# jynik/OOKiedokie

Hardware: AMD Instinct MI355X
Metric: IQ Msamples/s demodulated (SC16Q11->bits) (higher is better)
Workload: dtype f32

## Files before the change

### ookiedokie_amd/build.py

```python
from __future__ import annotations

import os
import shutil
import subprocess
import sys

HERE = os.path.dirname(os.path.abspath(__file__))
CSRC = os.path.join(HERE, "csrc")
LIB = os.path.join(HERE, "lib", "libookiedokie_amd.so")
SOURCES = ["loaders.cpp", "front_plan.cpp", "rx.cpp", "synth.cpp", "stream_fir.cpp", "backend.cpp", "edges_fsm.hip", "fsm_scan.hip",
           "formatter.cpp", "kernels.hip", "fir_mfma.hip", "fir_tuned.hip", "scan_ctx.cpp", "survey.cpp", "survey.hip",
           "survey_tuned.hip", "spectrum.cpp", "spectrum.hip", "pulses.cpp", "pulses.hip"]
ARCH = "gfx950"


def _hipcc() -> str:
    for cand in (shutil.which("hipcc"), "/opt/rocm/bin/hipcc"):
        if cand and os.path.exists(cand):
            return cand
    raise RuntimeError("hipcc not found")


def sources():
    return [os.path.join(CSRC, s) for s in SOURCES if os.path.exists(os.path.join(CSRC, s))]


def needs_build() -> bool:
    if not os.path.exists(LIB):
        return True
    t = os.path.getmtime(LIB)
    deps = sources() + [os.path.join(CSRC, f) for f in os.listdir(CSRC) if f.endswith(".hpp")]
    deps.append(os.path.join(HERE, "..", "include", "ookiedokie_amd.h"))
    return any(os.path.getmtime(d) > t for d in deps)


def build(force: bool = False, verbose: bool = False) -> str:
    if not force and not needs_build():
        return LIB
    os.makedirs(os.path.dirname(LIB), exist_ok=True)
    objs = []
    for src in sources():
        obj = os.path.join(HERE, "lib", os.path.basename(src) + ".o")
        cmd = [_hipcc(), "-x", "hip", "--offload-arch=" + ARCH, "-O3", "-std=c++17", "-fPIC",
               "-ffp-contract=off", "-fno-fast-math", "-Wall", "-Wno-unused-result", "-Wno-uninitialized",
               "-mllvm", "-amdgpu-atomic-optimizer-strategy=None",
               "-c", src, "-o", obj]
        if verbose:
            print(" ".join(cmd))
        r = subprocess.run(cmd, capture_output=True, text=True)
        if r.returncode != 0:
            raise RuntimeError("hipcc failed on %s:\n%s%s" % (src, r.stdout, r.stderr))
        if verbose and r.stderr:
            print(r.stderr)
        objs.append(obj)
    cmd = [_hipcc(), "--offload-arch=" + ARCH, "-shared", "-fPIC", "-o", LIB] + objs
    r = subprocess.run(cmd, capture_output=True, text=True)
    if r.returncode != 0:
        raise RuntimeError("link failed:\n%s%s" % (r.stdout, r.stderr))
    return LIB


if __name__ == "__main__":
    print(build(force="--force" in sys.argv, verbose=True))
```

### ookiedokie_amd/csrc/edges_fsm.hip

```cpp
#include "kernels.hpp"

namespace ookd {

__device__ __forceinline__ uint32_t lane_id() { return threadIdx.x & 63u; }

__device__ __forceinline__ uint32_t rfl(uint32_t v) {
    return (uint32_t)__builtin_amdgcn_readfirstlane((int)v);
}
__device__ __forceinline__ uint64_t rfl64(uint64_t v) {
    return ((uint64_t)rfl((uint32_t)(v >> 32)) << 32) | rfl((uint32_t)v);
}
__device__ __forceinline__ uint32_t rl(uint32_t v, uint32_t lane) {
    return (uint32_t)__builtin_amdgcn_readlane((int)v, (int)lane);
}
__device__ __forceinline__ uint64_t rl64(uint64_t v, uint32_t lane) {
    return ((uint64_t)rl((uint32_t)(v >> 32), lane) << 32) | rl((uint32_t)v, lane);
}


__device__ __forceinline__ uint64_t change_word(const uint64_t *words, uint64_t w, uint64_t n_out, uint32_t has_prev = 0) {
    const uint64_t cur = words[w];
    const uint64_t prev_top = (w == 0 && !has_prev) ? 0ull : (*(words + w - 1) >> 63);
    const uint64_t e = cur ^ ((cur << 1) | prev_top);
    const uint64_t base = w * 64;
// ... 67 lines not shown
#pragma unroll
    for (int d = 1; d < 64; d <<= 1) {
        const uint32_t t = __shfl_up(inc, d);
        if ((int)lane_id() >= d) inc += t;
    }
    if (lane_id() == 63) wave_sum[tid >> 6] = inc;
    __syncthreads();
    uint32_t before = 0;
    for (uint32_t w = 0; w < (tid >> 6); ++w) before += wave_sum[w];
    uint32_t run = before + inc - mine;
    if (quad && ((uintptr_t)(p.blk_offset + base) & 15u) == 0) {
        *reinterpret_cast<uint4 *>(p.blk_offset + base) = make_uint4(run, run + v[0], run + v[0] + v[1], run + v[0] + v[1] + v[2]);
        run += mine;
    } else {
#pragma unroll
        for (int i = 0; i < 4; ++i) {
            if (base + i < n) p.blk_offset[base + i] = run;
            run += v[i];
        }
    }
    if (tid == 255) p.group_total[blockIdx.x] = run;
}

__global__ __launch_bounds__(1024) void edge_scan_groups_kernel(const EdgeParams p) {
    __builtin_amdgcn_s_setprio(3);
    __shared__ uint32_t wtot[16];
    const uint32_t n = p.num_captures * p.blocks_per_cap;
    const uint32_t ng = (n + kScanGroup - 1) / kScanGroup;
    const uint32_t tid = threadIdx.x;
    const uint32_t chunk = (ng + 1023u) / 1024u;
    const uint32_t lo = min(tid * chunk, ng);
    const uint32_t hi = min(lo + chunk, ng);
    uint32_t sum = 0;
    for (uint32_t i = lo; i < hi; ++i) sum += p.group_total[i];
    uint32_t total = 0;
    uint32_t run = wg_inclusive_sum(sum, wtot, &total) - sum;
    for (uint32_t i = lo; i < hi; ++i) {
        const uint32_t t = p.group_total[i];
        p.group_total[i] = run;
        run += t;
    }
    if (tid == 1023) {
        p.blk_offset[n] = total;
        if ((uint64_t)total > p.edge_capacity) *p.overflow = 1;
        if (p.total_acc) atomicAdd(p.total_acc, total);
    }
}

constexpr uint32_t kWriteSpan = 4;

__global__ __launch_bounds__(256) void edge_write_kernel(const EdgeParams p) {
    __builtin_amdgcn_s_setprio(3);
    const uint32_t wave = (blockIdx.x * blockDim.x + threadIdx.x) >> 6;
    const uint32_t lane = lane_id();
    const uint32_t total_blocks = p.num_captures * p.blocks_per_cap;
    const uint32_t nwaves = (total_blocks + kWriteSpan - 1) / kWriteSpan;
    if (wave >= nwaves) return;
    uint32_t off = 0, cnt = 0;
    if (lane < kWriteSpan && wave + lane * nwaves < total_blocks) {
        const uint32_t b = wave + lane * nwaves;
        off = p.blk_offset[b] + p.group_total[b / kScanGroup];
        p.blk_offset[b] = off;
        cnt = p.blk_count[b];
    }
    uint64_t todo = __ballot(cnt != 0);
// ... 803 lines not shown
    }
    if (tid < p.hdr_words) {
        uint32_t v = p.d_hdr[tid];
        if (tid == p.edges_word && p.total_edges) v = *p.total_edges;
        p.h_hdr[tid] = v;
    }
    __syncthreads();
    if (tid < p.hdr_words) p.d_hdr[tid] = 0;
}

hipError_t launch_publish(const PublishParams &p, hipStream_t stream) {
    hipLaunchKernelGGL(publish_kernel, dim3(1), dim3(256), 0, stream, p);
    return hipGetLastError();
}


hipError_t launch_edges(const EdgeParams &p, hipStream_t stream) {
    const uint32_t total_blocks = p.num_captures * p.blocks_per_cap;
    if (total_blocks == 0) return hipSuccess;
    const uint32_t wgs = (total_blocks + 3) / 4;
    const uint32_t groups = (total_blocks + kScanGroup - 1) / kScanGroup;
    if (!p.tile_info) hipLaunchKernelGGL(edge_count_kernel, dim3(wgs), dim3(256), 0, stream, p);
    hipLaunchKernelGGL(edge_scan_local_kernel, dim3(groups), dim3(256), 0, stream, p);
    hipLaunchKernelGGL(edge_scan_groups_kernel, dim3(1), dim3(1024), 0, stream, p);
    if (p.tile_info) {
        const dim3 grid((uint32_t)(((uint64_t)total_blocks * p.tiles_per_block + 255) / 256));
        if (p.tiles_per_block == 4) hipLaunchKernelGGL(edge_write_tiles_kernel<4>, grid, dim3(256), 0, stream, p);
        else if (p.tiles_per_block == 8) hipLaunchKernelGGL(edge_write_tiles_kernel<8>, grid, dim3(256), 0, stream, p);
        else if (p.tiles_per_block == 16) hipLaunchKernelGGL(edge_write_tiles_kernel<16>, grid, dim3(256), 0, stream, p);
        else return hipErrorInvalidValue;
    } else {
        const uint32_t write_waves = (total_blocks + kWriteSpan - 1) / kWriteSpan;
        hipLaunchKernelGGL(edge_write_kernel, dim3((write_waves + 3) / 4), dim3(256), 0, stream, p);
    }
    return hipGetLastError();
}

hipError_t launch_fsm_prepare(const FsmParams &p, const FsmStateDev *first_state, hipStream_t stream) {
    const uint32_t nseg = p.num_captures * p.segs_per_cap;
    if (nseg == 0) return hipSuccess;
    FsmStateDev first{};
    if (first_state) first = *first_state;
    hipLaunchKernelGGL(fsm_cuts_kernel, dim3(p.num_captures * (p.segs_per_cap + 1)), dim3(64), 0, stream, p);
    hipLaunchKernelGGL(fsm_prepare_kernel, dim3((nseg + 63) / 64), dim3(64), 0, stream, p, first,
                       first_state ? 1 : 0);
    return hipGetLastError();
}
// ... 23 lines not shown
```

### ookiedokie_amd/csrc/fir_mfma.hip

```cpp
#include "kernels.hpp"
#include "common.hpp"

#include <hip/hip_ext.h>

#include <algorithm>
#include <cmath>
#include <cstring>
#include <type_traits>

#pragma clang fp contract(off)

namespace ookd {

typedef _Float16 h8 __attribute__((ext_vector_type(8)));
typedef _Float16 h4 __attribute__((ext_vector_type(4)));
typedef float f16x __attribute__((ext_vector_type(16)));
typedef float v2fm __attribute__((ext_vector_type(2)));
typedef short v2s __attribute__((ext_vector_type(2)));
typedef uint32_t v4u __attribute__((ext_vector_type(4)));

__host__ __device__ constexpr uint32_t mslot(uint32_t j) { return j + 8u * (j >> 5); }

template <int KS, int FMT = (int)kFmtSc16>
struct MfmaGeom {
// ... 505 lines not shown

        if (!more) break;
        if (!pre) mfma_boundary_loads<KS, FMT>(c, tile_n, tid, win, q);
        tile = tile_n;
    }
}

constexpr uint32_t kF2Out = 256;
constexpr uint32_t kF2Tp = 96;
constexpr uint32_t kF2W = 4 * kF2Out + kF2Tp;
template <int FMT>
struct F2Geom {
    static constexpr uint32_t vsamples = FMT == (int)kFmtSc16 ? 4u : 8u;
    static constexpr uint32_t nvec = kF2W / vsamples;
    static constexpr int rounds = (int)((nvec + 63) / 64);
};
constexpr int kF2KS = 5;
constexpr int kF2Waves = 4;
__host__ __device__ constexpr uint32_t f2slot(uint32_t j) { return j + 8u * (j >> 6); }
constexpr uint32_t kF2Plane = f2slot(kF2W) + 8u;
constexpr uint32_t kF2WaveBytes = kF2Plane * 2u * 2u;
constexpr uint32_t kF2ImgBytes = kF2KS * 2u * 1024u;
constexpr uint32_t kF2LdsBytes = kF2ImgBytes + kMfmaCtlBytes + kF2Waves * kF2WaveBytes;

typedef float f4x __attribute__((ext_vector_type(4)));

struct F2Taps {
    gptrf taps1, taps2;
    uint32_t n1, n2;
};

template <int FMT>
__device__ __forceinline__ float2 fir2_mfma_exact_output(const RawSrcT<FMT> &rs, const F2Taps &ft, int64_t m) {
    const float s = 1.0f / 2048.0f;
    float re2 = 0.0f, im2 = 0.0f;
    for (uint32_t k2 = 0; k2 < ft.n2; ++k2) {
        const int64_t j1 = 2 * m + 1 - (int64_t)k2;
        float re1 = 0.0f, im1 = 0.0f;
        for (uint32_t k1 = 0; k1 < ft.n1; ++k1) {
            const uint32_t w = fetch_raw_m(rs, 2 * j1 + 1 - (int64_t)k1);
            const float xr = (float)(int16_t)(w & 0xffffu) * s;
            const float xi = (float)(int16_t)(w >> 16) * s;
            const float t = ft.taps1[k1];
            const float pr = t * xr;
            const float pi = t * xi;
            re1 = re1 + pr;
// ... 532 lines not shown
```

### ookiedokie_amd/csrc/fsm_scan.hip

```cpp
#include "kernels.hpp"
#include "common.hpp"

#include <hip/hip_ext.h>

#include <algorithm>
#include <cstring>
#include <memory>
#include <vector>

namespace ookd {

namespace {

enum { kCondAlways = 1, kCondPulseStart, kCondPulseEnd, kCondTimeout, kCondMsgComplete };
enum { kActNone = 1, kActAppend0, kActAppend1, kActOutput };
enum { kResError = -1, kResNone = 0, kResOutput = 1 };

constexpr uint32_t kNone = 0xffffffffu;
constexpr uint32_t kSat = 0xfffffffeu;
constexpr uint32_t kMaxFires = 48;
constexpr uint32_t kMaxLeafApps = 30;
constexpr int kScanThreads = 1024;
constexpr uint32_t kStuckDepth = 8;
constexpr uint32_t kStuckDomain = 512;
// ... 292 lines not shown
    f.k = r.w[1];
    f.nbits = r.w[2];
    a.reset_seen = (r.w[0] >> 10) & 1u;
    a.sensitive = (r.w[0] >> 11) & 1u;
    a.overflow = (r.w[0] >> 12) & 1u;
    a.last_fired = (r.w[0] >> 14) & 1u;
    a.msgc_seen = (r.w[0] >> 13) & 1u;
    a.napp = r.w[3] & 0xffu;
    a.nout = (r.w[3] >> 8) & 0xffu;
    a.nerr = (r.w[3] >> 16) & 0xffu;
    a.apps_at_reset = r.w[3] >> 24;
    a.appvals = r.w[4];
    a.out_ab0 = r.w[5] & 0xffu;
    a.out_ab1 = (r.w[5] >> 8) & 0xffu;
    a.out_rb0 = (r.w[5] >> 16) & 0xffu;
    a.out_rb1 = r.w[5] >> 24;
    a.out_pos0 = r.w[6] | ((uint64_t)r.w[7] << 32);
    a.out_pos1 = r.w[8] | ((uint64_t)r.w[9] << 32);
    a.err_pos = r.w[10] | ((uint64_t)r.w[11] << 32);
    a.fires = 0;
    return (r.w[0] >> 9) & 1u;
}

__host__ __device__ __noinline__ SimRes run_leaf_raw(const LTab &T, uint32_t code, uint64_t pos0, uint64_t n, uint32_t lvl_edge,
                                            uint64_t resume, uint64_t prefix = 0) {
    const uint32_t NB1 = T.NB1;
    const uint32_t nstates = T.S * NB1;
    const uint32_t L = lvl_edge & 1u;
    const bool has_edge = (lvl_edge & 2u) != 0;
    PSim f;
    Acc a;
    acc_init(a);
    bool alive;
    if (code >= nstates) {
        f.cur = 0;
        f.nbits = 0;
        f.k = 0;
        f.prev = code - nstates;
        const uint64_t end_const = pos0 + n;
        const uint64_t last = end_const + (has_edge ? 1 : 0);
        if (resume >= last) alive = false;
        else if (resume >= end_const) alive = sim_span(T, f, a, resume, L, 0, has_edge);
        else alive = sim_span(T, f, a, resume, L, end_const - resume, has_edge);
    } else {
        f.cur = code / NB1;
        f.nbits = code - f.cur * NB1;
        f.k = 0;
        f.prev = L;
        bool lost = false;
        if (prefix) {
            lost = !sim_span(T, f, a, pos0 - prefix, L, prefix, false) || a.overflow;
            acc_init(a);
        }
        alive = sim_span(T, f, a, pos0, L, n, has_edge);
        if (lost) a.overflow = true;
    }
    return sim_pack(f, a, alive);
}

__device__ __forceinline__ bool run_leaf(const LTab &T, uint32_t code, const Span &sp, uint64_t resume, PSim &f,
                                         Acc &a) {
    const SimRes r = run_leaf_raw(T, code, sp.pos0, sp.n, sp.L | (sp.has_edge ? 2u : 0u), resume, sp.prefix);
    return sim_unpack(r, f, a);
}

__host__ __device__ __forceinline__ uint32_t encode_post(const LTab &T, const PSim &f, const Acc &a, bool alive) {
    if (a.overflow) return code_poison(T);
    if (!alive) return code_skip(T, f.prev);
    if (f.k != 0 && !(T.st[f.cur].w & 0x10000u)) return code_poison(T);
    return f.cur * T.NB1 + (f.nbits >= T.NB1 ? T.NB1 - 1 : f.nbits);
}

}

struct ScanParams {
    FsmParams f;
    uint16_t *block_tab;
    uint32_t *cap_block_off;
    LeafEvDev *events;
    uint8_t *app_vals;
    uint64_t app_capacity;
    uint64_t *errs;
    uint64_t err_capacity;
    FsmStateDev first;
    int have_first;
// ... 741 lines not shown
        STAMP(3);
#pragma unroll
        for (int j = 0; j < kIlp; ++j)
            if (valid[j]) row[code[j]] = (uint16_t)st[j];
    }
    STAMP(4);
    bool any = false;
    for (uint32_t w = 0; w < kCapWords; ++w) any = any || cap[w] != 0;
    if (any && T.NS) {
        const uint32_t nst = T.NS * T.depth;
        for (uint32_t item = threadIdx.x; item < nch * nst; item += blockDim.x) {
            const uint32_t c = item / nst, code = D0 + (item - c * nst);
            const uint32_t la = c * kChunk, lb = min((c + 1) * kChunk, count);
            const uint32_t ob = la + kStuckDepth - ((code - D0) / T.NS + 1);
            if (!(cap[ob >> 5] & (1u << (ob & 31u)))) continue;
            uint32_t v = code;
            for (uint32_t l = la; l < lb; ++l) v = leaf_step(T, sc, first, b.tab, rep, skip, SNB, l, v);
            b.ctab[c * D + code] = (uint16_t)v;
        }
    }
    __syncthreads();
}

__global__ __launch_bounds__(kScanThreads) void scan_layout_kernel(ScanParams sp) {
    __builtin_amdgcn_s_setprio(3);
    __shared__ uint32_t wtot[kScanThreads / 64];
    const uint32_t tid = threadIdx.x;
    const uint32_t nc = sp.f.num_captures;
    const uint32_t chunk = (nc + kScanThreads - 1) / kScanThreads;
    const uint32_t lo = min(tid * chunk, nc), hi = min(lo + chunk, nc);
    uint32_t sum = 0, sum2 = 0, sum3 = 0, sum4 = 0;
    for (uint32_t c = lo; c < hi; ++c) {
        uint64_t e0;
        const uint64_t ne = cap_edges(sp.f, c, e0);
        const uint64_t regular = ne > 1 ? ne - 1 : 0;
        const uint32_t nblk = (uint32_t)((regular + sp.leaf_block - 1) / sp.leaf_block);
        sum += nblk;
        sum2 += (uint32_t)((ne + 1 + kFinBlock - 1) / kFinBlock);
        sum3 += (nblk + 15u) / 16u;
        sum4 += (nblk + 63u) / 64u;
    }
    uint32_t tot = 0, tot2 = 0, tot3 = 0, tot4 = 0;
    uint32_t run = wg_inclusive_sum(sum, wtot, &tot) - sum;
    uint32_t run2 = wg_inclusive_sum(sum2, wtot, &tot2) - sum2;
    uint32_t run3 = wg_inclusive_sum(sum3, wtot, &tot3) - sum3;
    uint32_t run4 = wg_inclusive_sum(sum4, wtot, &tot4) - sum4;
    for (uint32_t c = lo; c < hi; ++c) {
        sp.cap_block_off[c] = run;
        sp.fin_off[c] = run2;
        sp.cap_group_off[c] = run3;
        sp.cap_super_off[c] = run4;
        uint64_t e0;
        const uint64_t ne = cap_edges(sp.f, c, e0);
        const uint64_t regular = ne > 1 ? ne - 1 : 0;
        const uint32_t nblk = (uint32_t)((regular + sp.leaf_block - 1) / sp.leaf_block);
        run += nblk;
        run2 += (uint32_t)((ne + 1 + kFinBlock - 1) / kFinBlock);
        run3 += (nblk + 15u) / 16u;
        run4 += (nblk + 63u) / 64u;
    }
    if (tid == kScanThreads - 1) {
        sp.cap_block_off[nc] = tot;
        sp.fin_off[nc] = tot2;
        sp.cap_group_off[nc] = tot3;
        sp.cap_super_off[nc] = tot4;
        if (tot > sp.total_blocks_cap || tot2 > sp.fin_blocks_cap) atomicOr(sp.fallback, (uint32_t)kFbBlocks);
        if (sp.edge_overflow && *sp.edge_overflow) atomicOr(sp.fallback, (uint32_t)kFbBlocks);
    }
}

__global__ __launch_bounds__(kSimThreads) void scan_leaf_kernel(ScanParams sp) {
    __builtin_amdgcn_s_setprio(3);
    __shared__ LTab T;
    __shared__ uint64_t s_resume[256];
    __shared__ uint16_t s_rep[256], s_uniq[258];
    __shared__ __attribute__((aligned(4))) uint16_t s_skip[256][2];
    __shared__ uint32_t s_cap[kCapWords];
    __shared__ uint32_t s_lt[kLtLdsWords];
    copy_ltab(T, sp.ltab);
    __syncthreads();
    if (threadIdx.x == 0) T.lvl0 = sp.has_prev ? fsm_level_at(sp.f, 0, -1) : 0u;
    __syncthreads();
    if (*sp.fallback) return;
    const uint32_t D = T.D, LB = sp.leaf_block;
// ... 1029 lines not shown
                    }
                }
            }
            if (bad && !stop && sp.f.debug) sp.f.debug[63] = gb | ((uint64_t)lb << 32);
            reinterpret_cast<uint16_t *>(rec + kSyncRecEnd)[k] = (uint16_t)s;
            if (bad) atomicOr(sp.sync_fail, 1u);
            mine = (arrive | (stop ? 0u : 4u)) << (3u * k);
        }
        mine |= (uint32_t)__shfl_xor((int)mine, 1);
        mine |= (uint32_t)__shfl_xor((int)mine, 2);
        mine |= (uint32_t)__shfl_xor((int)mine, 4);
        if (region && k == 0) sp.sync_dig[gb] = (info & 0x7fu) | 0x80u | (info & 0x700u) | (mine << kSyncDigMap);
    }
}

__device__ __forceinline__ uint32_t sync_map_identity() { return 0x03020100u; }
__device__ __forceinline__ uint32_t sync_map_apply(uint32_t m, uint32_t x) { return (m >> (8u * x)) & 0xffu; }
__device__ __forceinline__ uint32_t sync_map_then(uint32_t a, uint32_t b) {
    uint32_t r = 0;
#pragma unroll
    for (uint32_t x = 0; x < kSyncK; ++x) r |= sync_map_apply(b, sync_map_apply(a, x) & 3u) << (8u * x);
    return r;
}
constexpr uint32_t kPickPer = 32;

__device__ __forceinline__ uint32_t sync_dig_map(uint32_t dig) {
    const uint32_t mb = dig >> kSyncDigMap;
    return (mb & 3u) | (((mb >> 3) & 3u) << 8) | (((mb >> 6) & 3u) << 16) | (((mb >> 9) & 3u) << 24);
}

__global__ __launch_bounds__(kScanThreads) void scan_syncpick_kernel(ScanParams sp) {
    __builtin_amdgcn_s_setprio(3);
    __shared__ uint32_t maps[2][kScanThreads / 64];
    __shared__ uint32_t lastc[kScanThreads];
    uint32_t *const dig = reinterpret_cast<uint32_t *>(scan_smem);
    const uint32_t tid = threadIdx.x;
    if (*sp.fallback) return;
    if (*sp.sync_fail & 1u) {
        if (sp.sync_only && tid == 0) atomicOr(sp.fallback, (uint32_t)kFbSync);
        return;
    }
    for (uint32_t cap = blockIdx.x; cap < sp.f.num_captures; cap += gridDim.x) {
        const uint32_t gb0 = sp.cap_block_off[cap], nblk = sp.cap_block_off[cap + 1] - gb0;
        const uint32_t per = (nblk + kScanThreads - 1) / kScanThreads;
        if (per > kPickPer) {
            if (tid == 0) {
                atomicOr(sp.sync_fail, 1u);
                if (sp.sync_only) atomicOr(sp.fallback, (uint32_t)kFbSync);
            }
            return;
        }
        for (uint32_t i = tid; i < nblk; i += kScanThreads) dig[i] = sp.sync_dig[gb0 + i];
        __syncthreads();
        const uint32_t b0 = min(tid * per, nblk), b1 = min(b0 + per, nblk);
        uint32_t m = sync_map_identity();
        for (uint32_t b = b0; b < b1; ++b) {
            const uint32_t d = dig[b];
            if (d & 0x80u) m = sync_map_then(m, sync_dig_map(d));
        }
        const uint32_t lane = tid & 63u, wv = tid >> 6;
        uint32_t incl = m;
#pragma unroll
        for (uint32_t d = 1; d < 64; d <<= 1) {
            const uint32_t other = (uint32_t)__shfl_up((int)incl, (int)d);
            if (lane >= d) incl = sync_map_then(other, incl);
        }
        if (lane == 63) maps[0][wv] = incl;
        __syncthreads();
        if (wv == 0) {
            uint32_t t = lane < (uint32_t)(kScanThreads / 64) ? maps[0][lane] : sync_map_identity();
#pragma unroll
            for (uint32_t d = 1; d < (uint32_t)(kScanThreads / 64); d <<= 1) {
                const uint32_t other = (uint32_t)__shfl_up((int)t, (int)d);
                if (lane >= d) t = sync_map_then(other, t);
            }
            if (lane < (uint32_t)(kScanThreads / 64)) maps[1][lane] = t;
        }
        __syncthreads();
        uint32_t excl = (uint32_t)__shfl_up((int)incl, 1);
        if (lane == 0) excl = sync_map_identity();
        if (wv) excl = sync_map_then(maps[1][wv - 1], excl);
        uint32_t c = sync_map_apply(excl, 0u) & 3u;
        uint32_t last = 0xffffffffu;
        for (uint32_t b = b0; b < b1; ++b) {
            const uint32_t d = dig[b];
            if (d & 0x80u) {
                last = c;
                const uint32_t me = (d >> (kSyncDigMap + 3u * c)) & 7u;
                if (me & 4u) {
                    const uint32_t e = sp.sync_rec[(size_t)(gb0 + b) * kSyncRecWords + kSyncRecEnd + (c >> 1)];
                    sp.cap_end[cap] = (uint16_t)((e >> (16u * (c & 1u))) & 0xffffu);
                }
                dig[b] = (d & 0xffu) | (c << 12);
                c = me & 3u;
            } else {
                dig[b] = 64u;
            }
        }
        lastc[tid] = last;
        __syncthreads();
        uint32_t before = 0;
        if (b0 < b1) {
            for (uint32_t t = tid; t-- > 0;) {
                if (lastc[t] != 0xffffffffu) {
                    before = lastc[t];
                    break;
                }
            }
        }
        for (uint32_t b = b0; b < b1; ++b) {
            const uint32_t d = dig[b];
            dig[b] = (d & 0x7fu) | (before << 8) | (d & 0x3000u);
            if (d & 0x80u) before = (d >> 12) & 3u;
        }
        __syncthreads();
        for (uint32_t i = tid; i < nblk; i += kScanThreads) sp.sync_sel[gb0 + i] = dig[i];
        __syncthreads();
    }
}


__device__ __forceinline__ void emit_simulate(const ScanParams &sp, const LTab &T, uint32_t cap, const uint64_t *edges,
                                              size_t ev0, uint64_t i, uint32_t in) {
    const uint64_t e_before = edges[i - 1], e_at = edges[i];
    PSim f;
    Acc a;
    bool alive = true;
    if (in == code_poison(T)) {
        scan_refuse(sp, cap, (uint32_t)kFbPoison);
        acc_init(a);
        f.cur = f.nbits = f.k = f.prev = 0;
    } else {
        Span span;
        span.pos0 = e_before + 1;
        span.n = e_at - e_before - 1;
        span.L = (uint32_t)(i & 1ull) ^ T.lvl0;
        span.has_edge = true;
        span.prefix = 0;
        if (in >= T.S * T.NB1 + 3) {
            uint32_t d, src;
            stuck_decode(T, in, d, src);
            span.prefix = e_before - edges[i - d - 1];
            in = src;
        }
        alive = run_leaf(T, in, span, next_buffer_start(T, e_before), f, a);
        if (a.overflow) scan_refuse(sp, cap, (uint32_t)kFbOverflow);
    }
    put_event(sp, ev0 + i, a, f, alive, false);
}

constexpr uint32_t kEmitQueue = 1024;
struct EmitQ {
    uint32_t cap, in;
    uint64_t i;
};

__global__ __launch_bounds__(kSimThreads) void scan_emit_kernel(ScanParams sp) {
    __builtin_amdgcn_s_setprio(3);
    __shared__ LTab T;
    __shared__ EmitQ s_q[kEmitQueue];
    __shared__ uint32_t s_qn;
    copy_ltab(T, sp.ltab);
    __syncthreads();
    if (threadIdx.x == 0) {
        T.lvl0 = sp.has_prev ? fsm_level_at(sp.f, 0, -1) : 0u;
        s_qn = 0;
    }
    __syncthreads();
    if (*sp.fallback) return;
    const bool sync_form = sp.sync_try && !(*sp.sync_fail & 1u);
    const uint32_t LB = sp.leaf_block;
    const uint32_t total = sp.cap_block_off[sp.f.num_captures];
    if (sync_form) {
        const uint32_t r2 = sp.lt_merged[3] + 2u * (sp.lt_merged[0] + sp.lt_merged[1]);
        const uint32_t n2 = (sp.lt_merged[0] + sp.lt_merged[1]) * 2u * T.S;
        for (uint32_t i = threadIdx.x; i < n2; i += blockDim.x) g_mr[i] = sp.lt_merged[r2 + i];
        __syncthreads();
    }
    const uint32_t nquad = (total + 3u) / 4u;
    for (uint32_t wq = blockIdx.x; wq < nquad + sp.f.num_captures; wq += gridDim.x) {
// ... 81 lines not shown
                tail.prefix = 0;
                tail.pos0 = pos0;
                tail.n = sp.f.n_out > pos0 ? sp.f.n_out - pos0 : 0;
                tail.L = (uint32_t)(ne & 1ull) ^ T.lvl0;
                tail.has_edge = false;
                if (in > code_poison(T)) {
                    uint32_t d, src;
                    stuck_decode(T, in, d, src);
                    if (ne >= (uint64_t)d + 1) {
                        tail.prefix = edges[ne - 1] - edges[ne - d - 1];
                        in = src;
                    } else {
                        in = code_poison(T);
                    }
                }
                PSim f;
                Acc a;
                bool alive = true;
                if (in == code_poison(T)) {
                    scan_refuse(sp, cap, (uint32_t)kFbPoison);
                    acc_init(a);
                    f.cur = f.nbits = f.k = f.prev = 0;
                } else {
                    alive = run_leaf(T, in, tail, next_buffer_start(T, edges[ne - 1]), f, a);
                    if (a.overflow) scan_refuse(sp, cap, (uint32_t)kFbOverflow);
                }
                put_event(sp, ev0 + ne, a, f, alive, true);
            }
            __syncthreads();
        }
    }
    __syncthreads();
    const uint32_t nq = min(s_qn, kEmitQueue);
    for (uint32_t j = threadIdx.x; j < nq; j += blockDim.x) {
        const EmitQ e = s_q[j];
        uint64_t e0;
        (void)cap_edges(sp.f, e.cap, e0);
        emit_simulate(sp, T, e.cap, sp.f.edges + e0, (size_t)e0 + e.cap, e.i, e.in);
    }
}


__device__ __forceinline__ void locate_fin(const ScanParams &sp, uint32_t gfb, uint32_t &cap, uint32_t &fb) {
    uint32_t lo = 0, hi = sp.f.num_captures;
    while (hi - lo > 1) {
        const uint32_t mid = (lo + hi) >> 1;
        if (sp.fin_off[mid] <= gfb) lo = mid;
// ... 807 lines not shown
    sp.cap_super_off = a.cap_super_off;
    sp.super_tab = a.super_tab;
    sp.super_in = a.super_in;
    sp.sync_rec = a.sync_rec;
    sp.sync_dig = a.sync_rec ? a.sync_rec + (size_t)(a.total_blocks_cap + 8) * kSyncRecWords : nullptr;
    sp.sync_sel = a.sync_rec ? sp.sync_dig + a.total_blocks_cap + 8 : nullptr;
    sp.sync_fail = a.sync_fail;
    sp.sync_try = 0;
    sp.pre_plane = a.pre_plane;
    sp.lt_sync_words = a.lt_sync_words;
    sp.cap_end = a.cap_end;
    sp.cap_first = a.cap_first;
    const size_t lds = block_lds_bytes(a.leaf_block, a.D, a.S, a.SNB);
    const size_t lds_group = groups_lds_bytes(sp.Dp);
    const size_t lds_walk = (size_t)128 * sp.Dp * 2;
    if (lds_walk > 150u * 1024u) return hipErrorInvalidValue;
    hipError_t e;
    e = ensure_dynamic_lds(reinterpret_cast<const void *>(&scan_leaf_kernel), lds);
    if (e != hipSuccess) return e;
    e = ensure_dynamic_lds(reinterpret_cast<const void *>(&scan_walk_kernel), lds_walk);
    if (e != hipSuccess) return e;
    e = ensure_dynamic_lds(reinterpret_cast<const void *>(&scan_groups_kernel), lds_group);
    if (e != hipSuccess) return e;
    const size_t lds_pick = (size_t)kPickPer * kScanThreads * 4;
    e = ensure_dynamic_lds(reinterpret_cast<const void *>(&scan_syncpick_kernel), lds_pick);
    if (e != hipSuccess) return e;
    const char *const leaf_env = dev_getenv("OOKD_SCAN_LEAF");
    const size_t lds_wave = wave_lds_bytes(a.D, a.S);
    const bool wave_form = a.lt_off && a.lt_words && a.lt_words <= kLtLdsWords && a.leaf_block == 64 && lds_wave <= 60u * 1024u &&
                           !(leaf_env && leaf_env[0] == 'b');
    if (wave_form) {
        e = ensure_dynamic_lds(reinterpret_cast<const void *>(&scan_leaf_wave_kernel), lds_wave);
        if (e != hipSuccess) return e;
    }
    const uint32_t caps = a.f.num_captures;
    const uint32_t cap_grid = caps < 256 ? caps : 256;
    static thread_local int sim_dev = -1;
    static thread_local uint32_t leaf_grid = 0, emit_grid = 0, wave_grid = 0;
    static thread_local size_t wave_lds_seen = ~(size_t)0;
    if (wave_form) {
        int dev = 0;
        (void)hipGetDevice(&dev);
        if (dev != sim_dev || lds_wave != wave_lds_seen) {
            int per_cu = 0;
            hipDeviceProp_t prop;
            if (hipOccupancyMaxActiveBlocksPerMultiprocessor(&per_cu, scan_leaf_wave_kernel, 64, lds_wave) == hipSuccess &&
                hipGetDeviceProperties(&prop, dev) == hipSuccess && prop.multiProcessorCount > 0 && per_cu > 0) {
// ... 17 lines not shown
                hipGetDeviceProperties(&prop, dev) == hipSuccess && prop.multiProcessorCount > 0) {
                const int cus = prop.multiProcessorCount;
                leaf_grid = per_cu_leaf > 0 ? (uint32_t)(per_cu_leaf * cus) : a.grid_blocks;
                emit_grid = per_cu_emit > 0 ? (uint32_t)(per_cu_emit * cus) : a.grid_blocks;
            } else {
                (void)hipGetLastError();
                leaf_grid = emit_grid = a.grid_blocks;
            }
            sim_dev = dev;
            sim_lds = lds;
        }
    }
    static const char *const grid_env = dev_getenv("OOKD_SCAN_GRID");
    const uint32_t leaf_blocks = grid_env ? (uint32_t)atoi(grid_env) : leaf_grid;
    const uint32_t emit_blocks = grid_env ? (uint32_t)atoi(grid_env) : emit_grid;
    sp.skipc = wave_form ? a.skipc : nullptr;
    sp.skipc_valid = sp.skipc ? 1u : 0u;
    sp.pre_codes = a.pre_codes;
    sp.blk_in = a.blk_in;
    sp.rowz = a.rowz;
    sp.sync_try = (a.sync_try && wave_form && a.lt_merged && a.lt_sync_words && a.lt_sync_words <= kMergedLdsWords && a.rowz && a.skipc &&
                   a.pre_codes && a.pre_plane && a.sync_rec && a.sync_fail) ? 1u : 0u;
    sp.sync_only = sp.sync_try && a.sync_try == 2 ? 1u : 0u;
    hipLaunchKernelGGL(scan_layout_kernel, dim3(1), dim3(kScanThreads), 0, stream, sp);
    if (sp.sync_try) {
        hipLaunchKernelGGL(scan_sync_kernel, dim3(512), dim3(256), 0, stream, sp);
        hipLaunchKernelGGL(scan_syncwalk_kernel, dim3(512), dim3(256), 0, stream, sp);
        hipLaunchKernelGGL(scan_syncpick_kernel, dim3(cap_grid), dim3(kScanThreads), lds_pick, stream, sp);
    }
    if (!(sp.sync_try && sp.sync_only)) {
        if (wave_form) {
            hipLaunchKernelGGL(scan_leaf_wave_kernel, dim3(grid_env ? (uint32_t)atoi(grid_env) : wave_grid), dim3(64), lds_wave, stream, sp);
        } else {
            hipLaunchKernelGGL(scan_leaf_kernel, dim3(leaf_blocks), dim3(kSimThreads), lds, stream, sp);
        }
        hipLaunchKernelGGL(scan_groups_kernel, dim3(512), dim3(kGroupsThreads), lds_group, stream, sp);
        hipLaunchKernelGGL(scan_walk_kernel, dim3(cap_grid), dim3(kScanThreads), lds_walk, stream, sp);
        sp.entry_phase = 0;
        const bool with_phase2 = a.lt_off && a.lt_merged && a.rowz;
        hipLaunchKernelGGL(scan_entry_kernel, dim3(kEntryP0Blocks + (with_phase2 ? 512u : 0u)), dim3(256), 0, stream, sp);
        sp.entry_phase = 1;
        hipLaunchKernelGGL(scan_entry_kernel, dim3(512), dim3(256), 0, stream, sp);
    }
    hipLaunchKernelGGL(scan_emit_kernel, dim3(emit_blocks), dim3(kSimThreads), 0, stream, sp);
    hipLaunchKernelGGL(fin_write_kernel, dim3(256), dim3(kFinBlock), 0, stream, sp);
    hipExtLaunchKernelGGL(fin_msg_kernel, dim3(64), dim3(256), 0, stream, nullptr, t_end, 0, sp, a.publish);
    return hipGetLastError();
}

}
```

### ookiedokie_amd/csrc/kernels.hpp

```cpp
#pragma once

#include <hip/hip_runtime.h>

#include <vector>

#include <cstdint>

namespace ookd {

constexpr int kMaxStages = 8;
constexpr int kTapChunk = 32;
constexpr int kTunedChunk = 16;
constexpr int kFirThreads = 256;
constexpr int kFirR = 16;
constexpr int kFirTile = kFirThreads * kFirR;
constexpr int kFirWaves = kFirThreads / 64;
constexpr int kFirWgWaves = 1;
constexpr int kFir1RShort = 8, kFir1RLong = 16;
constexpr uint32_t kFir1ShortTaps = 256;
constexpr int kWaveTile = 64 * kFirR;
constexpr int kQuietCounters = 1024;
constexpr int kGenTile = 1024;
constexpr int kGenTileMin = 64;
constexpr size_t kGenLdsBytes = 160 * 1024;
// ... 114 lines not shown
bool front_uses_tuned_fir1(const FrontParams &p);
uint32_t tuned_fir1_tile_bits(const FrontParams &p);
hipError_t launch_front_tuned_fir1(const FrontParams &p, uint32_t num_captures, hipStream_t stream, hipEvent_t t0,
                                   hipEvent_t t1, uint64_t tile_begin, uint64_t tile_count);
hipError_t launch_front_tuned_generic(const FrontParams &p, uint32_t num_captures, hipStream_t stream);
constexpr uint32_t kMaxCarriers = 16;
struct TunedCarrierDev {
    uint32_t tap_off;
    float p_star, p_lo, p_hi;
    float quiet_a, quiet_b;
    uint32_t pad[2];
};
hipError_t launch_front_tuned_multi(const FrontParams &p, const TunedCarrierDev *carriers, uint32_t num_carriers,
                                    hipStream_t stream, hipEvent_t t0, hipEvent_t t1, uint64_t tile_begin,
                                    uint64_t tile_count);
hipError_t launch_front_generic(const FrontParams &p, uint32_t num_captures,
                                hipStream_t stream);
struct GenTile {
    uint32_t tile = 0;
    uint32_t lds_b_off = 0;
    uint64_t lds_bytes = 0;
};
GenTile generic_tile(const FirStageDev *stage, uint32_t num_stages);


constexpr int kScanGroup = 1024;

struct EdgeParams {
    const uint64_t *bits;
    uint64_t words_per_cap;
    uint64_t n_out;
    uint32_t num_captures;
    uint32_t blocks_per_cap;
    uint32_t *blk_count;
    uint32_t *blk_offset;
    uint32_t *group_total;
    uint64_t *edges;
    uint64_t edge_capacity;
    uint32_t *overflow;
    const uint32_t *tile_info;
    uint32_t tiles_per_block;
    uint32_t *total_acc;
    uint32_t has_prev;
    uint32_t stamp_bits;
};

// ... 170 lines not shown
    uint64_t pre_plane;
    uint32_t lt_sync_words;
    uint32_t *sync_fail;
    uint32_t sync_try;
};

constexpr uint32_t kScanFbSync = 16;
struct ScanTables {
    bool spans_built;
    uint32_t S, max_bits, NB1, SNB, D, leaf_block;
    std::vector<uint32_t> off, n0, pk;
    std::vector<uint16_t> reach;
    std::vector<uint16_t> reach_by_level;
    uint32_t reach_base, reach_lv[2];
    std::vector<uint16_t> stuck_src;
    std::vector<uint8_t> stuck_rows;
    std::vector<uint32_t> merged;
    uint32_t merged_rows_words;
    std::vector<uint4> ltab;
};
ScanTables build_scan_tables(const FsmTablesDev &tables, uint32_t spb, uint32_t decim, bool with_spans);
bool scan_tables_selfcheck(const ScanTables &t);
uint32_t fsm_scan_fin_block();
hipError_t launch_fsm_scan(const FsmScanArgs &a, hipStream_t stream, hipEvent_t t_end = nullptr);

#ifdef __HIPCC__
__device__ __forceinline__ uint32_t wg_inclusive_sum(uint32_t v, uint32_t *wtot, uint32_t *total) {
    const uint32_t lane = threadIdx.x & 63u, wave = threadIdx.x >> 6, nwaves = (blockDim.x + 63u) >> 6;
#pragma unroll
    for (int d = 1; d < 64; d <<= 1) {
        const uint32_t t = __shfl_up(v, d);
        if ((int)lane >= d) v += t;
    }
    __syncthreads();
    if (lane == 63u || threadIdx.x == blockDim.x - 1) wtot[wave] = v;
    __syncthreads();
    uint32_t before = 0, all = 0;
    for (uint32_t w = 0; w < nwaves; ++w) {
        const uint32_t t = wtot[w];
        if (w < wave) before += t;
        all += t;
    }
    if (total) *total = all;
    return v + before;
}
#endif
// ... 95 lines not shown
```

Measured before the change: 1.555 million.

## Shrink single-block scan kernels to a shared slot size so they co-reside with front-end

Introduces a 'slot' budget (256 threads, 128 VGPRs, LDS left after three front-end workgroups) and resizes the edge group scan, scan layout and sync-pick kernels from 1024/kScanThreads threads to this slot. Sync-pick is restructured into multiple passes with carried map state so its LDS footprint fits the slot, and scan_emit gets a VGPR cap. The intent is to let these small serial kernels run alongside front-end FIR work on the same CUs instead of needing a whole CU. The cost is less parallelism inside each of these kernels, possible register spills in scan_emit, and added carry logic across passes.

```diff
diff --git a/ookiedokie_amd/build.py b/ookiedokie_amd/build.py
--- a/ookiedokie_amd/build.py
+++ b/ookiedokie_amd/build.py
@@ -25,6 +25,12 @@
     return [os.path.join(CSRC, s) for s in SOURCES if os.path.exists(os.path.join(CSRC, s))]
 
 
+def compile_cmd():
+    return [_hipcc(), "-x", "hip", "--offload-arch=" + ARCH, "-O3", "-std=c++17", "-fPIC",
+            "-ffp-contract=off", "-fno-fast-math", "-Wall", "-Wno-unused-result", "-Wno-uninitialized",
+            "-mllvm", "-amdgpu-atomic-optimizer-strategy=None"]
+
+
 def needs_build() -> bool:
     if not os.path.exists(LIB):
         return True
@@ -41,10 +47,7 @@
     objs = []
     for src in sources():
         obj = os.path.join(HERE, "lib", os.path.basename(src) + ".o")
-        cmd = [_hipcc(), "-x", "hip", "--offload-arch=" + ARCH, "-O3", "-std=c++17", "-fPIC",
-               "-ffp-contract=off", "-fno-fast-math", "-Wall", "-Wno-unused-result", "-Wno-uninitialized",
-               "-mllvm", "-amdgpu-atomic-optimizer-strategy=None",
-               "-c", src, "-o", obj]
+        cmd = compile_cmd() + ["-c", src, "-o", obj]
         if verbose:
             print(" ".join(cmd))
         r = subprocess.run(cmd, capture_output=True, text=True)
diff --git a/ookiedokie_amd/csrc/edges_fsm.hip b/ookiedokie_amd/csrc/edges_fsm.hip
--- a/ookiedokie_amd/csrc/edges_fsm.hip
+++ b/ookiedokie_amd/csrc/edges_fsm.hip
@@ -113,13 +113,13 @@
     if (tid == 255) p.group_total[blockIdx.x] = run;
 }
 
-__global__ __launch_bounds__(1024) void edge_scan_groups_kernel(const EdgeParams p) {
+__global__ __launch_bounds__(kSlotThreads) void edge_scan_groups_kernel(const EdgeParams p) {
     __builtin_amdgcn_s_setprio(3);
-    __shared__ uint32_t wtot[16];
+    __shared__ uint32_t wtot[kSlotThreads / 64];
     const uint32_t n = p.num_captures * p.blocks_per_cap;
     const uint32_t ng = (n + kScanGroup - 1) / kScanGroup;
     const uint32_t tid = threadIdx.x;
-    const uint32_t chunk = (ng + 1023u) / 1024u;
+    const uint32_t chunk = (ng + kSlotThreads - 1u) / kSlotThreads;
     const uint32_t lo = min(tid * chunk, ng);
     const uint32_t hi = min(lo + chunk, ng);
     uint32_t sum = 0;
@@ -131,7 +131,7 @@
         p.group_total[i] = run;
         run += t;
     }
-    if (tid == 1023) {
+    if (tid == kSlotThreads - 1u) {
         p.blk_offset[n] = total;
         if ((uint64_t)total > p.edge_capacity) *p.overflow = 1;
         if (p.total_acc) atomicAdd(p.total_acc, total);
@@ -981,7 +981,7 @@
     const uint32_t groups = (total_blocks + kScanGroup - 1) / kScanGroup;
     if (!p.tile_info) hipLaunchKernelGGL(edge_count_kernel, dim3(wgs), dim3(256), 0, stream, p);
     hipLaunchKernelGGL(edge_scan_local_kernel, dim3(groups), dim3(256), 0, stream, p);
-    hipLaunchKernelGGL(edge_scan_groups_kernel, dim3(1), dim3(1024), 0, stream, p);
+    hipLaunchKernelGGL(edge_scan_groups_kernel, dim3(1), dim3(kSlotThreads), 0, stream, p);
     if (p.tile_info) {
         const dim3 grid((uint32_t)(((uint64_t)total_blocks * p.tiles_per_block + 255) / 256));
         if (p.tiles_per_block == 4) hipLaunchKernelGGL(edge_write_tiles_kernel<4>, grid, dim3(256), 0, stream, p);
diff --git a/ookiedokie_amd/csrc/fir_mfma.hip b/ookiedokie_amd/csrc/fir_mfma.hip
--- a/ookiedokie_amd/csrc/fir_mfma.hip
+++ b/ookiedokie_amd/csrc/fir_mfma.hip
@@ -551,6 +551,8 @@
 constexpr uint32_t kF2WaveBytes = kF2Plane * 2u * 2u;
 constexpr uint32_t kF2ImgBytes = kF2KS * 2u * 1024u;
 constexpr uint32_t kF2LdsBytes = kF2ImgBytes + kMfmaCtlBytes + kF2Waves * kF2WaveBytes;
+static_assert(kFront1WgLdsBytes == mfma_lds_bytes<4>() && mfma_waves<4>() == 4, "kernels.hpp: the slot's front-end term");
+static_assert(kFront2WgLdsBytes == kF2LdsBytes && kF2Waves == 4, "kernels.hpp: the slot's front-end term");
 
 typedef float f4x __attribute__((ext_vector_type(4)));
 
diff --git a/ookiedokie_amd/csrc/fsm_scan.hip b/ookiedokie_amd/csrc/fsm_scan.hip
--- a/ookiedokie_amd/csrc/fsm_scan.hip
+++ b/ookiedokie_amd/csrc/fsm_scan.hip
@@ -338,6 +338,7 @@
     return (r.w[0] >> 9) & 1u;
 }
 
+template <int kCopy = 0>
 __host__ __device__ __noinline__ SimRes run_leaf_raw(const LTab &T, uint32_t code, uint64_t pos0, uint64_t n, uint32_t lvl_edge,
                                             uint64_t resume, uint64_t prefix = 0) {
     const uint32_t NB1 = T.NB1;
@@ -374,9 +375,10 @@
     return sim_pack(f, a, alive);
 }
 
+template <int kCopy = 0>
 __device__ __forceinline__ bool run_leaf(const LTab &T, uint32_t code, const Span &sp, uint64_t resume, PSim &f,
                                          Acc &a) {
-    const SimRes r = run_leaf_raw(T, code, sp.pos0, sp.n, sp.L | (sp.has_edge ? 2u : 0u), resume, sp.prefix);
+    const SimRes r = run_leaf_raw<kCopy>(T, code, sp.pos0, sp.n, sp.L | (sp.has_edge ? 2u : 0u), resume, sp.prefix);
     return sim_unpack(r, f, a);
 }
 
@@ -1164,12 +1166,12 @@
     __syncthreads();
 }
 
-__global__ __launch_bounds__(kScanThreads) void scan_layout_kernel(ScanParams sp) {
+__global__ __launch_bounds__(kSlotThreads) void scan_layout_kernel(ScanParams sp) {
     __builtin_amdgcn_s_setprio(3);
-    __shared__ uint32_t wtot[kScanThreads / 64];
+    __shared__ uint32_t wtot[kSlotThreads / 64];
     const uint32_t tid = threadIdx.x;
     const uint32_t nc = sp.f.num_captures;
-    const uint32_t chunk = (nc + kScanThreads - 1) / kScanThreads;
+    const uint32_t chunk = (nc + kSlotThreads - 1) / kSlotThreads;
     const uint32_t lo = min(tid * chunk, nc), hi = min(lo + chunk, nc);
     uint32_t sum = 0, sum2 = 0, sum3 = 0, sum4 = 0;
     for (uint32_t c = lo; c < hi; ++c) {
@@ -1201,7 +1203,7 @@
         run3 += (nblk + 15u) / 16u;
         run4 += (nblk + 63u) / 64u;
     }
-    if (tid == kScanThreads - 1) {
+    if (tid == kSlotThreads - 1) {
         sp.cap_block_off[nc] = tot;
         sp.fin_off[nc] = tot2;
         sp.cap_group_off[nc] = tot3;
@@ -2277,17 +2279,23 @@
     for (uint32_t x = 0; x < kSyncK; ++x) r |= sync_map_apply(b, sync_map_apply(a, x) & 3u) << (8u * x);
     return r;
 }
-constexpr uint32_t kPickPer = 32;
+constexpr uint32_t kPickPer = 16;
+constexpr uint32_t kPickPass = kPickPer * kSlotThreads;
+constexpr uint32_t kPickMaxBlocks = 32u * 1024u;
+static_assert(kPickMaxBlocks % kPickPass == 0, "whole passes");
+size_t scan_syncpick_lds_bytes() { return (size_t)kPickPass * 4; }
 
 __device__ __forceinline__ uint32_t sync_dig_map(uint32_t dig) {
     const uint32_t mb = dig >> kSyncDigMap;
     return (mb & 3u) | (((mb >> 3) & 3u) << 8) | (((mb >> 6) & 3u) << 16) | (((mb >> 9) & 3u) << 24);
 }
 
-__global__ __launch_bounds__(kScanThreads) void scan_syncpick_kernel(ScanParams sp) {
+__global__ __launch_bounds__(kSlotThreads) void scan_syncpick_kernel(ScanParams sp) {
     __builtin_amdgcn_s_setprio(3);
-    __shared__ uint32_t maps[2][kScanThreads / 64];
-    __shared__ uint32_t lastc[kScanThreads];
+    constexpr uint32_t kWaves = kSlotThreads / 64;
+    __shared__ uint32_t maps[2][kWaves];
+    __shared__ uint32_t lastc[kSlotThreads];
+    __shared__ uint32_t s_carry[2];
     uint32_t *const dig = reinterpret_cast<uint32_t *>(scan_smem);
     const uint32_t tid = threadIdx.x;
     if (*sp.fallback) return;
@@ -2297,80 +2305,93 @@
     }
     for (uint32_t cap = blockIdx.x; cap < sp.f.num_captures; cap += gridDim.x) {
         const uint32_t gb0 = sp.cap_block_off[cap], nblk = sp.cap_block_off[cap + 1] - gb0;
-        const uint32_t per = (nblk + kScanThreads - 1) / kScanThreads;
-        if (per > kPickPer) {
+        if (nblk > kPickMaxBlocks) {
             if (tid == 0) {
                 atomicOr(sp.sync_fail, 1u);
                 if (sp.sync_only) atomicOr(sp.fallback, (uint32_t)kFbSync);
             }
             return;
         }
-        for (uint32_t i = tid; i < nblk; i += kScanThreads) dig[i] = sp.sync_dig[gb0 + i];
-        __syncthreads();
-        const uint32_t b0 = min(tid * per, nblk), b1 = min(b0 + per, nblk);
-        uint32_t m = sync_map_identity();
-        for (uint32_t b = b0; b < b1; ++b) {
-            const uint32_t d = dig[b];
-            if (d & 0x80u) m = sync_map_then(m, sync_dig_map(d));
-        }
-        const uint32_t lane = tid & 63u, wv = tid >> 6;
-        uint32_t incl = m;
-#pragma unroll
-        for (uint32_t d = 1; d < 64; d <<= 1) {
-            const uint32_t other = (uint32_t)__shfl_up((int)incl, (int)d);
-            if (lane >= d) incl = sync_map_then(other, incl);
-        }
-        if (lane == 63) maps[0][wv] = incl;
-        __syncthreads();
-        if (wv == 0) {
-            uint32_t t = lane < (uint32_t)(kScanThreads / 64) ? maps[0][lane] : sync_map_identity();
-#pragma unroll
-            for (uint32_t d = 1; d < (uint32_t)(kScanThreads / 64); d <<= 1) {
-                const uint32_t other = (uint32_t)__shfl_up((int)t, (int)d);
-                if (lane >= d) t = sync_map_then(other, t);
-            }
-            if (lane < (uint32_t)(kScanThreads / 64)) maps[1][lane] = t;
-        }
-        __syncthreads();
-        uint32_t excl = (uint32_t)__shfl_up((int)incl, 1);
-        if (lane == 0) excl = sync_map_identity();
-        if (wv) excl = sync_map_then(maps[1][wv - 1], excl);
-        uint32_t c = sync_map_apply(excl, 0u) & 3u;
-        uint32_t last = 0xffffffffu;
-        for (uint32_t b = b0; b < b1; ++b) {
-            const uint32_t d = dig[b];
-            if (d & 0x80u) {
-                last = c;
-                const uint32_t me = (d >> (kSyncDigMap + 3u * c)) & 7u;
-                if (me & 4u) {
-                    const uint32_t e = sp.sync_rec[(size_t)(gb0 + b) * kSyncRecWords + kSyncRecEnd + (c >> 1)];
-                    sp.cap_end[cap] = (uint16_t)((e >> (16u * (c & 1u))) & 0xffffu);
-                }
-                dig[b] = (d & 0xffu) | (c << 12);
-                c = me & 3u;
-            } else {
-                dig[b] = 64u;
-            }
-        }
-        lastc[tid] = last;
-        __syncthreads();
-        uint32_t before = 0;
-        if (b0 < b1) {
-            for (uint32_t t = tid; t-- > 0;) {
-                if (lastc[t] != 0xffffffffu) {
-                    before = lastc[t];
-                    break;
-                }
-            }
-        }
-        for (uint32_t b = b0; b < b1; ++b) {
-            const uint32_t d = dig[b];
-            dig[b] = (d & 0x7fu) | (before << 8) | (d & 0x3000u);
-            if (d & 0x80u) before = (d >> 12) & 3u;
-        }
-        __syncthreads();
-        for (uint32_t i = tid; i < nblk; i += kScanThreads) sp.sync_sel[gb0 + i] = dig[i];
-        __syncthreads();
+        if (tid == 0) {
+            s_carry[0] = sync_map_identity();
+            s_carry[1] = 0;
+        }
+        for (uint32_t p0 = 0; p0 < nblk; p0 += kPickPass) {
+            const uint32_t cnt = min(nblk - p0, kPickPass);
+            const uint32_t per = (cnt + kSlotThreads - 1) / kSlotThreads;
+            for (uint32_t i = tid; i < cnt; i += kSlotThreads) dig[i] = sp.sync_dig[gb0 + p0 + i];
+            __syncthreads();
+            const uint32_t b0 = min(tid * per, cnt), b1 = min(b0 + per, cnt);
+            uint32_t m = sync_map_identity();
+            for (uint32_t b = b0; b < b1; ++b) {
+                const uint32_t d = dig[b];
+                if (d & 0x80u) m = sync_map_then(m, sync_dig_map(d));
+            }
+            const uint32_t lane = tid & 63u, wv = tid >> 6;
+            uint32_t incl = m;
+#pragma unroll
+            for (uint32_t d = 1; d < 64; d <<= 1) {
+                const uint32_t other = (uint32_t)__shfl_up((int)incl, (int)d);
+                if (lane >= d) incl = sync_map_then(other, incl);
+            }
+            if (lane == 63) maps[0][wv] = incl;
+            __syncthreads();
+            if (wv == 0) {
+                uint32_t t = lane < kWaves ? maps[0][lane] : sync_map_identity();
+#pragma unroll
+                for (uint32_t d = 1; d < kWaves; d <<= 1) {
+                    const uint32_t other = (uint32_t)__shfl_up((int)t, (int)d);
+                    if (lane >= d) t = sync_map_then(other, t);
+                }
+                if (lane < kWaves) maps[1][lane] = t;
+            }
+            __syncthreads();
+            const uint32_t carry = s_carry[0], carry_before = s_carry[1];
+            uint32_t excl = (uint32_t)__shfl_up((int)incl, 1);
+            if (lane == 0) excl = sync_map_identity();
+            if (wv) excl = sync_map_then(maps[1][wv - 1], excl);
+            uint32_t c = sync_map_apply(sync_map_then(carry, excl), 0u) & 3u;
+            const uint32_t carry_next = sync_map_then(carry, maps[1][kWaves - 1]);
+            uint32_t last = 0xffffffffu;
+            for (uint32_t b = b0; b < b1; ++b) {
+                const uint32_t d = dig[b];
+                if (d & 0x80u) {
+                    last = c;
+                    const uint32_t me = (d >> (kSyncDigMap + 3u * c)) & 7u;
+                    if (me & 4u) {
+                        const uint32_t e = sp.sync_rec[(size_t)(gb0 + p0 + b) * kSyncRecWords + kSyncRecEnd + (c >> 1)];
+                        sp.cap_end[cap] = (uint16_t)((e >> (16u * (c & 1u))) & 0xffffu);
+                    }
+                    dig[b] = (d & 0xffu) | (c << 12);
+                    c = me & 3u;
+                } else {
+                    dig[b] = 64u;
+                }
+            }
+            lastc[tid] = last;
+            __syncthreads();
+            uint32_t before = carry_before;
+            if (b0 < b1) {
+                for (uint32_t t = tid; t-- > 0;) {
+                    if (lastc[t] != 0xffffffffu) {
+                        before = lastc[t];
+                        break;
+                    }
+                }
+            }
+            for (uint32_t b = b0; b < b1; ++b) {
+                const uint32_t d = dig[b];
+                dig[b] = (d & 0x7fu) | (before << 8) | (d & 0x3000u);
+                if (d & 0x80u) before = (d >> 12) & 3u;
+            }
+            if (b0 < b1 && b1 == cnt) {
+                s_carry[0] = carry_next;
+                s_carry[1] = before;
+            }
+            __syncthreads();
+            for (uint32_t i = tid; i < cnt; i += kSlotThreads) sp.sync_sel[gb0 + p0 + i] = dig[i];
+            __syncthreads();
+        }
     }
 }
 
@@ -2398,7 +2419,7 @@
             span.prefix = e_before - edges[i - d - 1];
             in = src;
         }
-        alive = run_leaf(T, in, span, next_buffer_start(T, e_before), f, a);
+        alive = run_leaf<1>(T, in, span, next_buffer_start(T, e_before), f, a);
         if (a.overflow) scan_refuse(sp, cap, (uint32_t)kFbOverflow);
     }
     put_event(sp, ev0 + i, a, f, alive, false);
@@ -2410,7 +2431,7 @@
     uint64_t i;
 };
 
-__global__ __launch_bounds__(kSimThreads) void scan_emit_kernel(ScanParams sp) {
+__global__ __launch_bounds__(kSimThreads) __attribute__((amdgpu_num_vgpr(kSlotVgprs))) void scan_emit_kernel(ScanParams sp) {
     __builtin_amdgcn_s_setprio(3);
     __shared__ LTab T;
     __shared__ EmitQ s_q[kEmitQueue];
@@ -2538,7 +2559,7 @@
                     acc_init(a);
                     f.cur = f.nbits = f.k = f.prev = 0;
                 } else {
-                    alive = run_leaf(T, in, tail, next_buffer_start(T, edges[ne - 1]), f, a);
+                    alive = run_leaf<1>(T, in, tail, next_buffer_start(T, edges[ne - 1]), f, a);
                     if (a.overflow) scan_refuse(sp, cap, (uint32_t)kFbOverflow);
                 }
                 put_event(sp, ev0 + ne, a, f, alive, true);
@@ -3392,7 +3413,7 @@
     if (e != hipSuccess) return e;
     e = ensure_dynamic_lds(reinterpret_cast<const void *>(&scan_groups_kernel), lds_group);
     if (e != hipSuccess) return e;
-    const size_t lds_pick = (size_t)kPickPer * kScanThreads * 4;
+    const size_t lds_pick = scan_syncpick_lds_bytes();
     e = ensure_dynamic_lds(reinterpret_cast<const void *>(&scan_syncpick_kernel), lds_pick);
     if (e != hipSuccess) return e;
     const char *const leaf_env = dev_getenv("OOKD_SCAN_LEAF");
@@ -3456,11 +3477,11 @@
     sp.sync_try = (a.sync_try && wave_form && a.lt_merged && a.lt_sync_words && a.lt_sync_words <= kMergedLdsWords && a.rowz && a.skipc &&
                    a.pre_codes && a.pre_plane && a.sync_rec && a.sync_fail) ? 1u : 0u;
     sp.sync_only = sp.sync_try && a.sync_try == 2 ? 1u : 0u;
-    hipLaunchKernelGGL(scan_layout_kernel, dim3(1), dim3(kScanThreads), 0, stream, sp);
+    hipLaunchKernelGGL(scan_layout_kernel, dim3(1), dim3(kSlotThreads), 0, stream, sp);
     if (sp.sync_try) {
         hipLaunchKernelGGL(scan_sync_kernel, dim3(512), dim3(256), 0, stream, sp);
         hipLaunchKernelGGL(scan_syncwalk_kernel, dim3(512), dim3(256), 0, stream, sp);
-        hipLaunchKernelGGL(scan_syncpick_kernel, dim3(cap_grid), dim3(kScanThreads), lds_pick, stream, sp);
+        hipLaunchKernelGGL(scan_syncpick_kernel, dim3(cap_grid), dim3(kSlotThreads), lds_pick, stream, sp);
     }
     if (!(sp.sync_try && sp.sync_only)) {
         if (wave_form) {
@@ -3483,3 +3504,12 @@
 }
 
 }
+
+extern "C" int ookd_chain_slot(uint32_t *out, uint32_t n) {
+    if (!out || n < 4) return -1;
+    out[0] = ookd::kSlotThreads;
+    out[1] = ookd::kSlotVgprs;
+    out[2] = ookd::kSlotLdsBytes;
+    out[3] = (uint32_t)ookd::scan_syncpick_lds_bytes();
+    return 0;
+}
diff --git a/ookiedokie_amd/csrc/kernels.hpp b/ookiedokie_amd/csrc/kernels.hpp
--- a/ookiedokie_amd/csrc/kernels.hpp
+++ b/ookiedokie_amd/csrc/kernels.hpp
@@ -160,6 +160,14 @@
     uint64_t lds_bytes = 0;
 };
 GenTile generic_tile(const FirStageDev *stage, uint32_t num_stages);
+
+constexpr uint32_t kCuLdsBytes = 160u * 1024u;
+constexpr uint32_t kFront1WgLdsBytes = 29328u;
+constexpr uint32_t kFront2WgLdsBytes = 30480u;
+constexpr uint32_t kSlotThreads = 256;
+constexpr uint32_t kSlotVgprs = 128;
+constexpr uint32_t kSlotLdsBytes =
+    kCuLdsBytes - 3u * (kFront1WgLdsBytes > kFront2WgLdsBytes ? kFront1WgLdsBytes : kFront2WgLdsBytes);
 
 
 constexpr int kScanGroup = 1024;
@@ -376,6 +384,7 @@
 ScanTables build_scan_tables(const FsmTablesDev &tables, uint32_t spb, uint32_t decim, bool with_spans);
 bool scan_tables_selfcheck(const ScanTables &t);
 uint32_t fsm_scan_fin_block();
+size_t scan_syncpick_lds_bytes();
 hipError_t launch_fsm_scan(const FsmScanArgs &a, hipStream_t stream, hipEvent_t t_end = nullptr);
 
 #ifdef __HIPCC__
```

Result: no change. 1.562 million, median of 3 (+0.5%).
